# ssttuu/go-pbrt

Measured on AMD Instinct MI355X. Metric: Mpaths/s (samples×pixels/s) at 1920×1080, 64 spp; 1/2/4/8-GPU scaling + HBM GB/s vs roofline, higher is better.
Workload: dtype f64

## Files before the change

go-pbrt_amd/csrc/k_chain.h:

```cpp
#pragma once
#pragma clang fp contract(off)

#include "render_common.h"

namespace pbrtk {

template <bool kX>
__device__ __forceinline__ uint32_t ring_d(const Cursor& c, const SpecSampler& ss, uint32_t d) {
    if (!kX || c.rri < 0 || d == kBadExactD || c.rrn == 0) return d;
    return kRrFlag | (d == kBadSpecD ? kRrTailBad : d);
}

__device__ __forceinline__ int uni(int v) { return __builtin_amdgcn_readfirstlane(v); }
__device__ __forceinline__ uint32_t uni(uint32_t v) { return (uint32_t)__builtin_amdgcn_readfirstlane((int)v); }
__device__ __forceinline__ float uni(float v) { return __int_as_float(__builtin_amdgcn_readfirstlane(__float_as_int(v))); }
__device__ __forceinline__ uint64_t uni(uint64_t v) {
    return (uint64_t)uni((uint32_t)(v >> 32)) << 32 | uni((uint32_t)v);
}
__device__ __forceinline__ int64_t uni(int64_t v) { return (int64_t)uni((uint64_t)v); }
__device__ __forceinline__ CiGroup uni(const CiGroup& s) {
    CiGroup u;
    u.S = uni(s.S);
    u.pi = uni(s.pi);
    u.npx = uni(s.npx);
    u.A = uni(s.A);
    u.head = uni(s.head);
    u.nxt = uni(s.nxt);
    u.kh = uni(s.kh);
    u.phase = uni(s.phase);
    u.reissue = uni(s.reissue);
    u.rb0 = uni(s.rb0);
    u.rb1 = uni(s.rb1);
    u.nb = uni(s.nb);
    u.nnx = uni(s.nnx);
    u.nps = uni(s.nps);
    u.dcnt = uni(s.dcnt);
    u.dsum = uni(s.dsum);
    u.dsq = uni(s.dsq);
    return u;
}

template <int kW, int kDepth, bool kX, int kEu, bool kSpWin, bool kMulti>
__global__ __launch_bounds__(kWave * kW) __attribute__((amdgpu_waves_per_eu(kEu > 0 ? kEu : kDepth < 0 ? PBRT_CI_MESH_EU_WAVES : kX ? PBRT_CI_X_EU_WAVES : PBRT_CI_EU_WAVES, 8))) void k_chain_ci(
    DevScene sc, RenderParams rp, ChainLayout lay, const PcgJump* __restrict__ jump, WaveBufs wb, int64_t slot_base,
    int64_t nslots_batch, int lanes_per_tile, int ring_size, Counters* __restrict__ ctr,
    const uint32_t* __restrict__ order, uint32_t* __restrict__ ticks, int cstride, uint32_t* __restrict__ prog) {
    extern __shared__ __attribute__((aligned(16))) unsigned char lds[];
    const uint64_t t_begin = wall_clock64();
    if (prog && threadIdx.x == 0) __hip_atomic_fetch_add(&prog[0], 1u, __ATOMIC_RELAXED, __HIP_MEMORY_SCOPE_AGENT);
    const uint32_t cs = cstride == 1 ? 1u : 2u;
    constexpr int kT = kWave * kW;
    __shared__ uint16_t stack_lds[kDepth > 0 ? kDepth * kT : 1];
#ifdef PBRT_CI_DENSE_WALK
    __shared__ __attribute__((aligned(16))) unsigned char dense_lds[kDepth > 0 ? 16 : kW * kDenseScratch];
#endif
    __shared__ CiGroup gs[kCiMaxGroups];
    __shared__ uint64_t sh_state;
    __shared__ uint32_t sh_draws;
    __shared__ int sh_act;
    __shared__ int wcnt[kW];
#ifdef PBRT_CI_DIAG
    __shared__ uint32_t dh[64];
#endif
    static_assert(!kMulti || kW == 1, "several tiles per wave: one-wave workgroups only");
    const int tid = threadIdx.x, lane = tid & (kWave - 1), wv = kW > 1 ? uni(tid / kWave) : 0;
    stage_nodes(sc);
    const int L = kMulti ? lanes_per_tile : kT, G = kMulti ? kWave / L : 1;
    const int g = kMulti ? lane / L : 0, gl = kMulti ? lane - g * L : tid;
    const int64_t blk = order ? (int64_t)order[blockIdx.x] : (int64_t)blockIdx.x;
    const uint32_t R = (uint32_t)ring_size;
    const PcgJump& J = *jump;
    double* s1d = lay.s1d >= 0 ? (double*)(lds + lay.s1d) : nullptr;
    uint16_t* other = (uint16_t*)(lds + lay.other);
    uint32_t* vbuf = (uint32_t*)(lds + lay.vbuf);
    constexpr bool kNps = kW > 1 && !kX;
    const bool nps_on = kNps && rp.ci_nps != 0 && cstride == 1;
    constexpr uint32_t kNpsMinStats = 16;
    constexpr bool kStats = !kX && (kW > 1 || kDepth < 0);
    const float zcap = nps_on ? 3.0f : rp.ci_scap >= 0 ? 0.1f * (float)rp.ci_scap : kDepth < 0 ? 1.5f : 0.0f;
    auto ring_of = [&](int64_t pix) -> RingEnt* {
        return (RingEnt*)(lds + lay.ring) + (size_t)(nps_on ? (int)(pix & 1) : g) * R;
    };
    auto rpar = [&](int64_t pix) -> int { return nps_on ? (int)(pix & 1) : 0; };
    ChainCache* pcs = (ChainCache*)(lds + lay.pcs);
    uint16_t* stack = stack_lds + tid;
    const int n = rp.spp, ndims = rp.ndims;
#ifndef PBRT_CI_TAILCAP
#define PBRT_CI_TAILCAP 1
#endif
    const uint32_t dmax = (uint32_t)(camera_draws(ndims) + 8 * (rp.max_depth + 1) + 8);
    const pbrt_camera_desc& cam = *sc.camera;
    const unsigned long long gmask = !kMulti || L >= 64 ? ~0ULL : (((1ULL << (L & 63)) - 1ULL) << (g * L));
    const int64_t bs = blk * G + g;
    const uint64_t inc = pcg_inc_of((uint64_t)tile_of_slot(rp, slot_base + (bs < nslots_batch ? bs : 0)));
#ifdef PBRT_CI_DIAG
    unsigned long long steps = 0, busy = 0;
    unsigned long long ph_cyc[8] = {0, 0, 0, 0, 0, 0, 0, 0};
    long long tprev = clock64();
    auto mark = [&](int k) {
        long long now = clock64();
        ph_cyc[k] += (unsigned long long)(now - tprev);
        tprev = now;
    };
    if (tid < 64) dh[tid] = 0;
#define CI_DIAG(x) x
#else
    auto mark = [](int) {};
#define CI_DIAG(x)
#endif
    if (tid < G) {
        const int64_t b = blk * G + tid;
        CiGroup& s = gs[tid];
        s.pi = 0;
        s.kh = 1;
        s.A = s.head = s.nxt = 0;
        s.rb0 = s.rb1 = 0;
        s.nb = s.nnx = 0;
        s.nps = 0;
        s.dcnt = 0;
        s.dsum = s.dsq = 0.0f;
        s.reissue = 0;
        if (b < nslots_batch) {
            int64_t x0, y0, x1, y1;
            tile_bounds(rp, tile_of_slot(rp, slot_base + b), x0, y0, x1, y1);
            Pcg seed;
            pcg_seed(seed, (uint64_t)tile_of_slot(rp, slot_base + b));
            s.S = seed.state;
            s.npx = (x1 - x0) * (y1 - y0);
            s.phase = s.npx > 0 ? 0 : 2;
            wb.tile_npx[b] = 0;
        } else {
            s.S = 0;
            s.npx = 0;
            s.phase = 2;
        }
    }
    __syncthreads();

    uint32_t cancel_poll = 0;
    uint64_t last_host_poll = t_begin;
    uint32_t off = kNoOff;
    int opi_r = -1;
#ifdef PBRT_CI_LDS_STATE
    constexpr bool kLdsState = true;
#else
    constexpr bool kLdsState = kX;
#endif
    __shared__ Spec xs_beta[kLdsState ? kT : 1];
    __shared__ double xs_eta[kLdsState ? kT : 1];
    constexpr bool kStIssue = !kMulti;
    __shared__ uint64_t xs_st0[kLdsState && !kStIssue ? kT : 1];
    uint64_t st0_r = 0;
    Spec beta_r = spec(1);
    double eta_r = 1.0;
    uint64_t& st0 = [&]() -> uint64_t& { if constexpr (kLdsState && !kStIssue) return xs_st0[tid]; else return st0_r; }();
    Spec& beta = [&]() -> Spec& { if constexpr (kLdsState) return xs_beta[tid]; else return beta_r; }();
    double& eta_scale = [&]() -> double& { if constexpr (kLdsState) return xs_eta[tid]; else return eta_r; }();
    st0 = 0;
    beta = spec(1);
    eta_scale = 1.0;
    bool tracing = false;
    Cursor c;
    c.rri = -1;
    c.rrn = 0;
    c.rng.state = 0;
    c.rng.inc = inc;
    c.draws = 0;
    c.cur1d = c.cur2d = 0;
    c.k = -1;
    c.kdep = 0;
    int bounces = 1;
    Ray ray;
    ray.o = ray.d = V3{0, 0, 0};
    ray.tmax = kInf;
    ray.time = 0;

    CiGroup sg;
    if constexpr (kMulti) sg = gs[g];
    else sg = uni(gs[0]);
    int64_t rec = bs * wb.ppt + sg.pi;
    SpecSampler ss{wb.s1d + rec * wb.s1d_stride, n, ndims, kX && wb.rrb ? wb.rrb + bs * kCiMaxRing : nullptr};

    constexpr bool kOneScatter = kDepth >= 0 && !kSpWin;
    using Both = std::integral_constant<int, 0>;
    using Fresh = std::integral_constant<int, 1>;
    using Hits = std::integral_constant<int, 2>;
    int best = -1;
    V3 ph{0, 0, 0};
    auto traverse = [&]() __attribute__((always_inline)) {
        const int64_t opi = kNps ? (int64_t)opi_r : sg.pi;
        best = -1;
        int panic = 0;
#ifdef PBRT_CI_DENSE_WALK
        const bool dense = kDepth == 0 && sc.dense_ok && sc.use_lds_nodes;
        if (dense) bvh_walk_dense(sc, ray, tracing, panic, best, ph, dense_lds + (size_t)wv * kDenseScratch);
        if (tracing) {
            if (!dense) bvh_walk<false, kT, PBRT_CHAIN_LB, (kDepth < 0)>(sc, ray, stack, panic, best, ph);
#else
        if (tracing) {
            bvh_walk<false, kT, PBRT_CHAIN_LB, (kDepth < 0)>(sc, ray, stack, panic, best, ph);
#endif
            if (panic || best < 0) {
                RingEnt& e = ring_of(opi)[(off - (rpar(opi) ? sg.rb1 : sg.rb0)) & (R - 1u)];
                if constexpr (!kStIssue) e.st = st0;
                e.d = ring_d<kX>(c, ss, panic ? (c.k >= 0 ? kBadExactD : kBadSpecD) : c.draws);
                e.tag = off;
                off = kNoOff;
                tracing = false;
            }
        }
    };
    auto scatter = [&](auto which, bool fresh) __attribute__((always_inline)) {
        constexpr int kWhich = decltype(which)::value;
        const bool first = kWhich == Fresh::value ? true : kWhich == Hits::value ? false : fresh;
        if (kWhich == Fresh::value ? fresh : kWhich == Hits::value ? tracing : (fresh || tracing)) {
            const int64_t spi = kNps ? (int64_t)opi_r : sg.pi;
            SI si;
            BSDF b;
            BSDFX x;
            V3 wo = ray.d;
            bool ok = true;
            if (first) {
                const ChainCache& pc = pcs[2 * g + rpar(spi)];
                si = pc.si;
                b = pc.b;
                if constexpr (kX) x = pc.x;
                wo = pc.wo;
            } else {
                prim_si(sc, best, ray, ph, si);
                ok = (kX ? compute_bsdf_x(sc, si, b, x) : compute_bsdf(sc, si, b)) >= 0;
            }
            const int r = !ok ? 2
                              : traj_scatter<kX>(sc, si, b, x, wo, c, ss, beta, eta_scale, bounces, ray, rp.max_depth,
                                                 rp.rr_threshold);
            tracing = r == 0;
            if (r != 0) {
                RingEnt& e = ring_of(spi)[(off - (rpar(spi) ? sg.rb1 : sg.rb0)) & (R - 1u)];
                if constexpr (!kStIssue) e.st = st0;
                e.d = ring_d<kX>(c, ss, r == 1 ? c.draws : (c.k >= 0 ? kBadExactD : kBadSpecD));
                e.tag = off;
                off = kNoOff;
            }
        }
    };
    auto walk_drop = [&]() __attribute__((always_inline)) {
        const int64_t opi = kNps ? (int64_t)opi_r : sg.pi;
        __syncthreads();
        if (gl == 0 && sg.phase == 1) {
            CiGroup s = gs[g];
            if ((++cancel_poll & 127u) == 0) {
                const uint64_t now = wall_clock64();
                const bool host = now - last_host_poll >= 100000;
                if (host) last_host_poll = now;
                if (cancel_requested(sc, host)) s.phase = 2;
            }
            RingEnt* rcur = ring_of(s.pi);
            const uint32_t rbase = rpar(s.pi) ? s.rb1 : s.rb0;
            for (; s.phase == 1;) {
                RingEnt& e = rcur[(s.head - rbase) & (R - 1u)];
                if (e.tag != s.head) break;
                uint32_t d = e.d;
                if (kX && d < kBadExactD && (d & kRrFlag)) {
                    const RrBranches& b = ss.rrb[(s.head - rbase) & (R - 1u)];
                    d = (d & kRrTailBad) == kRrTailBad ? kBadSpecD : (d & kRrTailBad);
                    for (uint32_t i = 0; i < b.n; i++) {
                        const uint32_t cd = b.cd[i];
                        if (ss.s1d[(int)(cd & 0xFFu) * n + s.kh] < b.q[i]) {
                            d = cd >> 8;
                            break;
                        }
                    }
                }
                if (d == kBadSpecD) {
                    e.tag = kNoOff;
                    s.reissue = 1;
                    break;
                }
                wb.memb[rec * n + s.kh] = e.st;
                if (d == kBadExactD) {
                    wb.prec[rec].nvalid = s.kh + 1;
                    s.phase = 2;
                    break;
                }
                CI_DIAG(atomicAdd(&dh[min(d / 2u, 63u)], 1u);)
                CI_DIAG(if (d > dmax) ph_cyc[6]++;)
                CI_DIAG(if (d & 1u) atomicAdd(&ctr->odd_d, 1ull);)
                if (kStats) {
                    s.dcnt++;
                    s.dsum += (float)d;
                    s.dsq += (float)d * (float)d;
                }
                s.kh++;
                s.head += d;
                if (s.kh >= n) {
                    s.S = pcg_advance(J, s.S, inc, (uint64_t)(s.head - s.A));
                    s.A = s.head;
                    s.pi++;
                    s.phase = s.pi < s.npx ? 0 : 2;
                    break;
                }
            }
            if (s.nxt < s.head || (cs == 2u && ((s.nxt ^ s.head) & 1u))) s.nxt = s.head;
            int act = 0;
            const int left = n - s.kh;
            const bool stats = s.dcnt >= kNpsMinStats;
            if (nps_on && s.phase == 1 && !s.nps && (left == 1 || (stats && left <= rp.ci_nps)) &&
                s.pi + 1 < s.npx) {
                const PixelRec& pn = wb.prec[rec + 1];
                if (pn.hit && !pn.panic0) {
                    float lo = 0.0f;
                    if (left > 1) {
                        const float mu = s.dsum / (float)s.dcnt;
                        const float sd = sqrtf(fmaxf(0.0f, s.dsq / (float)s.dcnt - mu * mu));
                        lo = fmaxf(0.0f, (float)left * mu - 3.0f * sd * sqrtf((float)left));
                    }
                    s.nps = 1;
                    s.nb = s.head + (uint32_t)lo + (uint32_t)rp.sp_events;
                    s.nnx = s.nb;
                    if (rpar(s.pi + 1)) s.rb1 = s.nb;
                    else s.rb0 = s.nb;
                    act = 1;
                }
            }
            if (kNps) sh_act = act;
            CiGroup& gw = gs[g];
            gw.S = s.S;
            gw.A = s.A;
            gw.pi = s.pi;
            gw.head = s.head;
            gw.nxt = s.nxt;
            gw.kh = s.kh;
            gw.phase = s.phase;
            gw.reissue = s.reissue;
            if (kStats) {
                gw.dcnt = s.dcnt;
                gw.dsum = s.dsum;
                gw.dsq = s.dsq;
            }
            if (kNps) {
                gw.nps = s.nps;
                gw.nb = s.nb;
                gw.nnx = s.nnx;
                gw.rb0 = s.rb0;
                gw.rb1 = s.rb1;
            }
        }
        if (kNps && tid == 0 && !(gl == 0 && sg.phase == 1)) sh_act = 0;
        __syncthreads();
        if (kNps && sh_act) {
            const CiGroup s3 = uni(gs[0]);
            RingEnt* rn = ring_of(s3.pi + 1);
            for (uint32_t i = (uint32_t)tid; i < R; i += kT) rn[i].tag = kNoOff;
            if (tid == 0) {
                const PixelRec& pn = wb.prec[rec + 1];
                ChainCache& pc = pcs[2 * g + rpar(s3.pi + 1)];
                pc.si = pn.si;
                pc.b = pn.b;
                pc.wo = pn.wo;
                pc.hit = pn.hit;
            }
        }
        if (off != kNoOff) {
            const CiGroup s2 = gs[g];
            bool keep = false;
            if ((!kNps || opi == s2.pi) && s2.phase == 1)
                keep = !(off < s2.head || (cs == 2u && ((off ^ s2.head) & 1u)) ||
                         (PBRT_CI_TAILCAP && off > s2.head + (uint32_t)(n - 1 - s2.kh) * dmax));
            else if (kNps && opi == s2.pi && s2.phase == 0)
                keep = s2.nps != 0;
            else if (kNps && opi == s2.pi + 1 && s2.phase == 1)
                keep = s2.nps != 0;
            if (!keep) {
                off = kNoOff;
                tracing = false;
            }
        }
    };

    for (;;) {
        if constexpr (kOneScatter) {
            CI_DIAG(const unsigned long long tbusy = __ballot(tracing); if (lane == 0) busy += (unsigned long long)__popcll(tbusy);)
            traverse();
            mark(2);
            walk_drop();
            mark(4);
        }
        for (int q = 0; q < G; q++) {
            while (gs[q].phase == 0) {
                const int64_t bq = blk * G + q;
                const int64_t tile = tile_of_slot(rp, slot_base + bq);
                const uint64_t incq = pcg_inc_of((uint64_t)tile);
                const int64_t pi = gs[q].pi;
                const int64_t rec = bq * wb.ppt + pi;
                int64_t x0, y0, x1, y1;
                tile_bounds(rp, tile, x0, y0, x1, y1);
                const int64_t px = x0 + pi % (x1 - x0), py = y0 + pi / (x1 - x0);
                double* gs1d = wb.s1d + rec * wb.s1d_stride;
                double* sp = s1d ? s1d : gs1d;
                uint64_t S1;
                [[clang::always_inline]] S1 = start_pixel_wave<kSpWin>(rp, J, gs[q].S, incq, sp, other, vbuf, &sh_state, &sh_draws);
                if (s1d)
                    for (int idx = tid; idx < ndims * n; idx += kT) gs1d[idx] = s1d[idx];
                const double time_u = sp[1 < n ? 1 : 0];
                __syncthreads();
                const bool spec_ran = nps_on && gs[q].nps != 0;
                if (!spec_ran) {
                    RingEnt* rq = nps_on ? ring_of(pi) : (RingEnt*)(lds + lay.ring) + (size_t)q * R;
                    for (uint32_t i = (uint32_t)tid; i < R; i += kT) rq[i].tag = kNoOff;
                }
                PixelRec& pr = wb.prec[rec];
                const int hit0 = pr.hit, panic0 = pr.panic0;
                if (tid == 0) {
                    if (prog)
                        __hip_atomic_fetch_add(&prog[2], 1u, __ATOMIC_RELAXED, __HIP_MEMORY_SCOPE_AGENT);
                    const uint64_t now = wall_clock64();
                    const bool host = now - last_host_poll >= 100000;
                    if (host) last_host_poll = now;
                    if (cancel_requested(sc, host))
                        for (int q2 = 0; q2 < G; q2++) gs[q2].phase = 2;
                }
                if (tid == 0 && gs[q].phase == 0) {
                    if (hit0)
                        pr.si.time = camera_ray(cam, (double)px, (double)py, time_u, V2{0.0, 0.0}).time;
                    ChainCache& pq = pcs[2 * q + rpar(pi)];
                    pq.si = pr.si;
                    pq.b = pr.b;
                    if constexpr (kX) pq.x = pr.x;
                    pq.wo = pr.wo;
                    pq.hit = hit0;
                    CiGroup& s = gs[q];
                    s.S = S1;
                    s.A += sh_draws;
                    s.head = s.A;
                    s.nxt = (spec_ran && s.A >= s.nb) ? max(s.nnx, s.A) : s.A;
                    if (!spec_ran) {
                        if (rpar(pi)) s.rb1 = s.A;
                        else s.rb0 = s.A;
                    }
                    s.nps = 0;
                    s.kh = 1;
                    s.reissue = 0;
                    wb.tile_npx[bq] = (int32_t)(pi + 1);
                    if (panic0) {
                        s.phase = 2;
                    } else if (hit0) {
                        s.phase = 1;
                    } else {
                        if (ndims < 2) {
                            s.S = pcg_advance(J, S1, incq, (uint64_t)(n - 1) * camera_draws(ndims));
                            s.A += (uint32_t)(n - 1) * camera_draws(ndims);
                        }
                        s.pi = pi + 1;
                        s.phase = s.pi < s.npx ? 0 : 2;
                    }
                }
                __syncthreads();
            }
        }
        mark(0);
        bool any_chain = false;
        for (int q = 0; q < G; q++) any_chain |= gs[q].phase == 1;
        if (!any_chain) break;
        CI_DIAG(steps++;)

        if constexpr (kMulti) sg = gs[g];
        else sg = uni(gs[0]);
        rec = bs * wb.ppt + sg.pi;
        ss.s1d = wb.s1d + rec * wb.s1d_stride;
        bool fresh = false;
        {
            const bool idle = sg.phase == 1 && off == kNoOff;
            const unsigned long long m = __ballot(idle) & gmask;
            int nidle = __popcll(m);
            int rank;
            if constexpr (kMulti) rank = __popcll(m & ((1ULL << lane) - 1ULL));
            else rank = (int)__builtin_amdgcn_mbcnt_hi((uint32_t)(m >> 32), __builtin_amdgcn_mbcnt_lo((uint32_t)m, 0u));
            if (kW > 1) {
                if (lane == 0) wcnt[wv] = nidle;
                __syncthreads();
                int before = 0, tot = 0;
                for (int w = 0; w < kW; w++) {
                    const int cw = wcnt[w];
                    before += w < wv ? cw : 0;
                    tot += cw;
                }
                rank += before;
                nidle = tot;
            }
            const int re = (sg.reissue && nidle > 0) ? 1 : 0;
            const uint32_t nx0 = sg.nxt;
            const int avail = nx0 < sg.head + R ? (int)((sg.head + R - nx0 + cs - 1) / cs) : 0;
#if PBRT_CI_TAILCAP
            const uint32_t tail = sg.head + (uint32_t)(n - 1 - sg.kh) * dmax;
            const int capn = nx0 <= tail ? (int)((tail - nx0) / cs) + 1 : 0;
            int nspec = min(min(nidle - re, avail), capn);
            if (kStats && zcap > 0.0f && sg.dcnt >= kNpsMinStats) {
                const float rem = (float)(n - 1 - sg.kh);
                const float mu = sg.dsum / (float)sg.dcnt;
                const float sd = sqrtf(fmaxf(0.0f, sg.dsq / (float)sg.dcnt - mu * mu));
                const uint32_t scap = sg.head + (uint32_t)(rem * mu + zcap * sd * sqrtf(rem));
                nspec = min(nspec, nx0 <= scap ? (int)((scap - nx0) / cs) + 1 : 0);
            }
#else
            const int nspec = min(nidle - re, avail);
#endif
            int nspec1 = 0;
            if (kNps && sg.phase == 1 && sg.nps) {
                const int avail1 = sg.nnx < sg.nb + R ? (int)(sg.nb + R - sg.nnx) : 0;
                nspec1 = max(0, min(nidle - re - max(nspec, 0), avail1));
            }
            uint32_t o = kNoOff;
            bool exact = false;
            int opix = (int)sg.pi;
            if (idle) {
                if (re && rank == 0) {
                    o = sg.head;
                    exact = true;
                } else {
                    rank -= re;
                    if (rank < nspec) {
                        o = nx0 + cs * (uint32_t)rank;
                    } else if (kNps && rank - nspec < nspec1) {
                        o = sg.nnx + (uint32_t)(rank - nspec);
                        opix = (int)sg.pi + 1;
                    }
                }
            }
            if (gl == 0 && sg.phase == 1) {
                gs[g].nxt = nx0 + cs * (uint32_t)max(nspec, 0);
                if (kNps) gs[g].nnx = sg.nnx + (uint32_t)nspec1;
                CI_DIAG(ph_cyc[5] += (unsigned long long)(max(nspec, 0) + nspec1 + re);)
                CI_DIAG(ph_cyc[7] += (unsigned long long)nspec1;)
                if (re) gs[g].reissue = 0;
            }
            if (o != kNoOff) {
                off = o;
                if (kNps) opi_r = opix;
                RingEnt& e = ring_of(opix)[(off - (rpar(opix) ? sg.rb1 : sg.rb0)) & (R - 1u)];
                if constexpr (kStIssue) {
                    const uint64_t st = pcg_advance(J, sg.S, inc, (uint64_t)(o - sg.A));
                    e.st = st;
                    c.rng.state = st;
                } else {
                    st0 = pcg_advance(J, sg.S, inc, (uint64_t)(o - sg.A));
                    c.rng.state = st0;
                }
                c.draws = 0;
                c_camera(c, ndims);
                c.k = exact ? sg.kh : -1;
                c.kdep = 0;
                if constexpr (kX) {
                    c.rri = (!exact && ss.rrb) ? (int)((off - sg.rb0) & (R - 1u)) : -1;
                    c.rrn = 0;
                }
                beta = spec(1);
                eta_scale = 1.0;
                bounces = 1;
                fresh = true;
            }
        }
        if constexpr (kOneScatter) {
            mark(1);
            scatter(Both{}, fresh);
            mark(3);
        } else {
            scatter(Fresh{}, fresh);
            mark(1);
            CI_DIAG(const unsigned long long tbusy = __ballot(tracing); if (lane == 0) busy += (unsigned long long)__popcll(tbusy);)
            traverse();
            mark(2);
            scatter(Hits{}, false);
            mark(3);
            walk_drop();
            mark(4);
        }
    }
#ifdef PBRT_CI_DIAG
    __syncthreads();
    if (tid < 64 && dh[tid]) atomicAdd(&ctr->dhist[tid], (unsigned long long)dh[tid]);
    if (tid == 0) {
        atomicAdd(&ctr->windows, steps);
        for (int k = 0; k < 8; k++) atomicAdd(&ctr->phase[k], ph_cyc[k]);
        atomicAdd(&ctr->nps_issued, ph_cyc[7]);
    }
    if (lane == 0) atomicAdd(&ctr->busy, busy);
#endif
#undef CI_DIAG
    if (prog) {
        __threadfence();
        __syncthreads();
    }
    if (tid == 0) {
        if (prog && G == 1 && bs < nslots_batch) {
// ... 16 lines not shown
```

go-pbrt_amd/csrc/k_chain_c.hip:

```cpp
#pragma clang fp contract(off)

#include "render_common.h"
#include "cam_sample.h"
#include "k_chain.h"

namespace pbrtk {

#ifndef PBRT_CAM_EU_WAVES
#define PBRT_CAM_EU_WAVES 3
#endif

struct CamGroup {
    uint64_t S;
    int64_t pi;
    int64_t npx;
    uint32_t A;
    uint32_t head;
    uint32_t nxt;
    int kh;
    int phase;
    int px, py;
};

__global__ __launch_bounds__(kWave) __attribute__((amdgpu_waves_per_eu(PBRT_CAM_EU_WAVES, 8))) void k_chain_cam(
    DevScene sc, RenderParams rp, ChainLayout lay, const PcgJump* __restrict__ jump, WaveBufs wb, int64_t slot_base,
    int64_t nslots_batch, const uint32_t* __restrict__ order, uint32_t* __restrict__ ticks) {
    extern __shared__ __attribute__((aligned(16))) unsigned char lds[];
    const uint64_t t_begin = wall_clock64();
    __shared__ uint16_t stack_lds[1];
    __shared__ CamGroup gs;
    __shared__ uint64_t sh_state;
    __shared__ uint32_t sh_draws;
    const int tid = threadIdx.x;
    stage_nodes(sc);
    const int64_t bs = order ? (int64_t)order[blockIdx.x] : (int64_t)blockIdx.x;
    if (bs >= nslots_batch) return;
    constexpr uint32_t R = kCiRingBytes / sizeof(RingEnt);
    const PcgJump& J = *jump;
    double* s1d = lay.s1d >= 0 ? (double*)(lds + lay.s1d) : nullptr;
    uint16_t* other = (uint16_t*)(lds + lay.other);
    uint32_t* vbuf = (uint32_t*)(lds + lay.vbuf);
    RingEnt* ring = (RingEnt*)(lds + lay.ring);
    uint16_t* stack = stack_lds + tid;
    const int n = rp.spp, ndims = rp.ndims;
    const uint32_t dmax = pbrtcam::cam_draws(ndims) + (uint32_t)(8 * (rp.max_depth + 1) + 8);
    const pbrt_camera_desc& cam = *sc.camera;
    const int64_t tile = tile_of_slot(rp, slot_base + bs);
    const uint64_t inc = pcg_inc_of((uint64_t)tile);
    int64_t x0, y0, x1, y1;
    tile_bounds(rp, tile, x0, y0, x1, y1);
    if (tid == 0) {
        Pcg seed;
        pcg_seed(seed, (uint64_t)tile);
        gs.S = seed.state;
        gs.pi = 0;
        gs.npx = (x1 - x0) * (y1 - y0);
        gs.A = gs.head = gs.nxt = 0;
        gs.kh = 1;
        gs.phase = (gs.npx > 0 && n > 1) ? 0 : 2;
        gs.px = gs.py = 0;
        wb.tile_npx[bs] = 0;
    }
    __syncthreads();

    uint32_t cancel_poll = 0;
    uint64_t last_host_poll = t_begin;
    uint32_t off = kNoOff;
    bool tracing = false;
    Cursor c;
    c.rri = -1;
    c.rrn = 0;
    c.rng.state = 0;
    c.rng.inc = inc;
    c.draws = 0;
    c.cur1d = c.cur2d = 0;
    c.k = -1;
    c.kdep = 0;
    Spec beta = spec(1);
    double eta_scale = 1.0;
    int bounces = 1;
    Ray ray;
    ray.o = ray.d = V3{0, 0, 0};
    ray.tmax = kInf;
    ray.time = 0;
    const SpecSampler ss{nullptr, n, ndims, nullptr};

    auto finish = [&](uint32_t d) {
        RingEnt& e = ring[off & (R - 1u)];
        e.d = d;
        e.tag = off;
        off = kNoOff;
        tracing = false;
    };

    for (;;) {
        if (tracing) {
            int panic = 0, best = -1;
            V3 ph{0, 0, 0};
            bvh_walk<false, kWave, PBRT_CHAIN_LB, false>(sc, ray, stack, panic, best, ph);
            if (panic || best < 0) {
                finish(panic ? kBadExactD : c.draws);
            } else {
                SI si;
                BSDF b;
                BSDFX x;
                const V3 wo = ray.d;
                prim_si(sc, best, ray, ph, si);
                const int r = compute_bsdf(sc, si, b) < 0
                                  ? 2
                                  : traj_scatter<false>(sc, si, b, x, wo, c, ss, beta, eta_scale, bounces, ray,
                                                        rp.max_depth, rp.rr_threshold);
                if (r != 0) finish(r == 1 ? c.draws : kBadExactD);
            }
        }
        __syncthreads();
        if (tid == 0 && gs.phase == 1) {
            CamGroup s = gs;
            if ((++cancel_poll & 127u) == 0) {
                const uint64_t now = wall_clock64();
                const bool host = now - last_host_poll >= 100000;
                if (host) last_host_poll = now;
                if (cancel_requested(sc, host)) s.phase = 2;
            }
            const int64_t rec = bs * wb.ppt + s.pi;
            for (; s.phase == 1;) {
                const RingEnt& e = ring[s.head & (R - 1u)];
                if (e.tag != s.head) break;
                const uint32_t d = e.d;
                wb.memb[rec * n + s.kh] = e.st;
                if (d == kBadExactD) {
                    wb.prec[rec].nvalid = s.kh + 1;
                    s.phase = 2;
                    break;
                }
                s.kh++;
                s.head += d;
                if (s.kh >= n) {
                    s.S = pcg_advance(J, s.S, inc, (uint64_t)(s.head - s.A));
                    s.A = s.head;
                    s.pi++;
                    s.phase = s.pi < s.npx ? 0 : 2;
                    break;
                }
            }
            if (s.nxt < s.head) s.nxt = s.head;
            gs.S = s.S;
            gs.A = s.A;
            gs.pi = s.pi;
            gs.head = s.head;
            gs.nxt = s.nxt;
            gs.kh = s.kh;
            gs.phase = s.phase;
        }
        __syncthreads();
        if (off != kNoOff) {
            const uint32_t head = uni(gs.head);
            const bool keep = uni(gs.phase) == 1 && off >= head && off <= head + (uint32_t)(n - 1 - uni(gs.kh)) * dmax;
            if (!keep) {
                off = kNoOff;
                tracing = false;
            }
        }
        while (gs.phase == 0) {
            const int64_t pi = gs.pi;
            const int64_t rec = bs * wb.ppt + pi;
            uint64_t S1 = gs.S;
            uint32_t sp_draws = 0;
            if (ndims > 0) {
                double* gs1d = wb.s1d + rec * wb.s1d_stride;
                [[clang::always_inline]] S1 = start_pixel_wave<false>(rp, J, gs.S, inc, s1d ? s1d : gs1d, other, vbuf, &sh_state, &sh_draws);
                sp_draws = sh_draws;
                if (s1d)
                    for (int idx = tid; idx < ndims * n; idx += kWave) gs1d[idx] = s1d[idx];
            }
            __syncthreads();
            for (uint32_t i = (uint32_t)tid; i < R; i += kWave) ring[i].tag = kNoOff;
            if (tid == 0) {
                const uint64_t now = wall_clock64();
                const bool host = now - last_host_poll >= 100000;
                if (host) last_host_poll = now;
                PixelRec& pr = wb.prec[rec];
                pr.hit = 1;
                pr.panic0 = 0;
                pr.nvalid = n;
                wb.tile_npx[bs] = (int32_t)(pi + 1);
                gs.S = S1;
                gs.A += sp_draws;
                gs.head = gs.nxt = gs.A;
                gs.kh = 1;
                gs.px = (int)(x0 + pi % (x1 - x0));
                gs.py = (int)(y0 + pi / (x1 - x0));
                gs.phase = cancel_requested(sc, host) ? 2 : 1;
            }
            __syncthreads();
        }
        if (gs.phase != 1) break;

        {
            const uint32_t head = uni(gs.head), nx0 = uni(gs.nxt), A = uni(gs.A);
            const int kh = uni(gs.kh);
            const uint64_t S = uni(gs.S);
            const int px = uni(gs.px), py = uni(gs.py);
            const bool idle = off == kNoOff;
            const unsigned long long m = __ballot(idle);
            const int nidle = __popcll(m);
            const int rank = (int)__builtin_amdgcn_mbcnt_hi((uint32_t)(m >> 32), __builtin_amdgcn_mbcnt_lo((uint32_t)m, 0u));
            const int avail = nx0 < head + R ? (int)(head + R - nx0) : 0;
            const uint32_t tail = head + (uint32_t)(n - 1 - kh) * dmax;
            const int capn = nx0 <= tail ? (int)(tail - nx0) + 1 : 0;
            const int nspec = min(min(nidle, avail), capn);
            if (tid == 0) gs.nxt = nx0 + (uint32_t)nspec;
            if (idle && rank < nspec) {
                off = nx0 + (uint32_t)rank;
                uint64_t st = pcg_advance(J, S, inc, (uint64_t)(off - A));
                ring[off & (R - 1u)].st = st;
                const pbrtcam::CamSample cs = pbrtcam::cam_sample(st, inc, ndims);
                c.rng.state = st;
                c.draws = cs.draws;
                c.cur1d = ndims < 1 ? ndims : 1;
                c.cur2d = ndims < 2 ? ndims : 2;
                c.kdep = 0;
                beta = spec(1);
                eta_scale = 1.0;
                bounces = 1;
                if (bounces >= rp.max_depth) {
                    finish(c.draws);
                } else {
                    ray = camera_ray(cam, (double)px + cs.film_x, (double)py + cs.film_y, cs.time_u,
                                     V2{cs.lens_x, cs.lens_y});
                    tracing = true;
                }
            }
        }
    }
    if (tid == 0 && ticks) {
        const uint64_t t_end = wall_clock64();
        ticks[bs] = (uint32_t)min(t_end - t_begin, (uint64_t)0xFFFFFFFFu);
    }
}

}
```

go-pbrt_amd/csrc/pbrt_spec.h:

```cpp
#pragma once
#pragma clang fp contract(off)

#include "pbrt_path.h"
#include <type_traits>

namespace pbrt {

struct PcgJump {
    uint64_t a[64];
    uint64_t b[64];
};
__device__ __forceinline__ uint64_t pcg_advance(const PcgJump& J, uint64_t s, uint64_t inc, uint64_t n) {
    for (int i = 0; n; ++i, n >>= 1)
        if (n & 1) s = J.a[i] * s + inc * J.b[i];
    return s;
}
__device__ __forceinline__ uint32_t pcg_output(uint64_t old) {
    uint32_t xs = (uint32_t)(((old >> 18) ^ old) >> 27);
    uint32_t rot = (uint32_t)(old >> 59);
    return (xs >> rot) | (xs << ((rot + 1u) & 31u));
}

constexpr int kRrBranches = 3;
struct RrBranches {
    double q[kRrBranches];
    uint32_t cd[kRrBranches];
    uint32_t n;
};
struct SpecSampler {
    const double* s1d;
    int spp, ndims;
    RrBranches* rrb;
};
struct Cursor {
    Pcg rng;
    uint32_t draws;
    int cur1d, cur2d;
    int k;
    int kdep;
    int rri;
    int rrn;
};
__device__ __forceinline__ double c_get1d(Cursor& c, const SpecSampler& s) {
    if (c.cur1d < s.ndims) {
        const int d = c.cur1d++;
        if (c.k < 0) {
            c.kdep = 1;
            return 0.5;
        }
        return s.s1d[d * s.spp + c.k];
    }
    c.draws++;
    return pcg_float(c.rng);
}
__device__ __forceinline__ void c_skip1d(Cursor& c, const SpecSampler& s) {
    if (c.cur1d < s.ndims) {
        c.cur1d++;
        return;
    }
    c.draws++;
    pcg_next(c.rng);
}
__device__ __forceinline__ V2 c_get2d(Cursor& c, const SpecSampler& s) {
    if (c.cur2d < s.ndims) {
        c.cur2d++;
        return V2{0.0, 0.0};
    }
    c.draws += 2;
    double x = pcg_float(c.rng);
// ... 153 lines not shown
        if (kX && type == -1) {
            panic = PBRT_PANIC_NIL_DEREF;
            return true;
        }
        if (is_black(f) || pdf == 0.0) {
            done = true;
        } else {
            double wp = absdot(wi, isect.sn) / pdf;
            s.beta = smul(s.beta, smuls(f, wp));
            if (kX && (type & BXDF_SPECULAR) && (type & BXDF_TRANSMISSION)) {
                const double eta = x.eta;
                if (dot(wo, isect.n) > 0) s.eta_scale *= eta * eta;
                else s.eta_scale *= 1 / (eta * eta);
            }
            s.ray.o = offset_ray_origin(isect.p, isect.perr, isect.n, wi);
            s.ray.d = wi;
            s.ray.tmax = kInf;
            s.ray.time = isect.time;
            Spec rr = smuls(s.beta, kX ? s.eta_scale : 1.0);
            if (max_component(rr) < rr_threshold && s.bounces > 3) {
                double q = gomath::max(0.05, 1 - max_component(rr));
                double u1 = c_get1d(c, ss);
                if (c.kdep || u1 < q) done = true;
                else s.beta = sdivs(s.beta, 1 - q);
            }
        }
    }
    if (pending) {
        Spec ld = spec(0);
        if (shadow) {
            add_rays(s, kRayShadow);
            const bool occluded = bvh_traverse<true, PBRT_PATHS_LB>(sc, sr, nullptr, stack, panic);
            if (panic) return true;
            if (!occluded) {
                if constexpr (kLdsAux) ld = s.aux[1];
                else ld = ld_vis;
            }
        }
        if (max_component(ld) > 10) {
            panic = PBRT_PANIC_LD_GT_10;
            return true;
        }
        if constexpr (kLdsAux) beta0 = s.aux[0];
        add_L(s, smul(beta0, ld));
    }
    return done;
}

template <bool kX = false>
__device__ inline int traj_scatter(const DevScene& sc, const SI& isect, const BSDF& b, const BSDFX& x, V3 wo,
                                   Cursor& c, const SpecSampler& ss, Spec& beta, double& eta_scale, int& bounces,
                                   Ray& ray, int max_depth, double rr_threshold) {
    if ((kX ? bsdfx_nonspecular(b, x) : b.n_bxdfs > 0) && sc.n_lights > 0) {
        c_skip1d(c, ss);
        c_get2d(c, ss);
        c_get2d(c, ss);
    }
    V2 u = c_get2d(c, ss);
    V3 wi;
    double pdf;
    int type = 0;
    Spec f = kX ? bsdfx_sample_f(b, x, wo, u, wi, pdf, type) : bsdf_sample_f(b, wo, u, wi, pdf);
    if (kX && type == -1) return 2;
    if (is_black(f) || pdf == 0.0) return 1;
    double wp = absdot(wi, isect.sn) / pdf;
    beta = smul(beta, smuls(f, wp));
    if (kX && (type & BXDF_SPECULAR) && (type & BXDF_TRANSMISSION)) {
        const double eta = x.eta;
        if (dot(wo, isect.n) > 0) eta_scale *= eta * eta;
        else eta_scale *= 1 / (eta * eta);
    }
    ray.o = offset_ray_origin(isect.p, isect.perr, isect.n, wi);
    ray.d = wi;
    ray.tmax = kInf;
    ray.time = isect.time;
    Spec rr = smuls(beta, kX ? eta_scale : 1.0);
    if (max_component(rr) < rr_threshold && bounces > 3) {
        double q = gomath::max(0.05, 1 - max_component(rr));
        if (kX && c.k < 0 && c.rri >= 0 && c.cur1d < ss.ndims) {
            RrBranches& rb = ss.rrb[c.rri];
            if (c.rrn == kRrBranches || c.draws >= (1u << 24)) return 2;
            rb.q[c.rrn] = q;
            rb.cd[c.rrn] = (c.draws << 8) | (uint32_t)c.cur1d;
            rb.n = (uint32_t)++c.rrn;
            c.cur1d++;
            beta = sdivs(beta, 1 - q);
        } else {
            double u1 = c_get1d(c, ss);
            if (c.kdep) return 2;
            if (u1 < q) return 1;
            beta = sdivs(beta, 1 - q);
        }
    }
    bounces++;
    return bounces >= max_depth ? 1 : 0;
}

}
```

go-pbrt_amd/csrc/render.hip:

```cpp
#pragma clang fp contract(off)

#include <hip/hip_runtime.h>

#include <algorithm>
#include <atomic>
#include <chrono>
#include <cstdio>
#include <cstring>
#include <string>
#include <functional>
#include <mutex>
#include <unordered_map>
#include <vector>

#include "../../include/pbrt_gpu.h"
#include "../../include/pbrt_diag.h"
#include "../../include/pbrt_scene.h"
#include "mesh_bvh.h"
#include "query_buffers.h"
#include "render_kernels.h"

using namespace pbrt;
using namespace pbrtk;

// ... 436 lines not shown
        v[i].prim_to_world = p.prim_to_world;
        v[i].kind = p.kind;
        v[i].material = p.material;
        v[i].prim_identity = is_identity(p.prim_to_world.m) ? 1 : 0;
        v[i].fast = xf_fast_kind(p.prim_to_world.m_inv) | xf_fast_kind(v[i].shape.object_to_world.m_inv) << 8;
    }
    return v;
}

int validate_scene(const pbrt_scene_desc* s) {
    if (!s) return PBRT_E_INVALID;
    if (s->n_prims < 0 || s->n_nodes < 0 || s->n_lights < 0 || s->n_shapes < 0 || s->n_materials < 0)
        return PBRT_E_INVALID;
    if (s->n_nodes > 32767) return PBRT_E_UNSUPPORTED;
    for (int i = 0; i < s->n_prims; i++) {
        const pbrt_primitive_desc& p = s->prims[i];
        if (p.shape < 0 || p.shape >= s->n_shapes || p.material < 0 || p.material >= s->n_materials)
            return PBRT_E_INVALID;
        if (p.kind != PBRT_PRIM_GEOMETRIC && p.kind != PBRT_PRIM_TRANSFORMED) return PBRT_E_INVALID;
    }
    for (int i = 0; i < s->n_shapes; i++)
        if (s->shapes[i].type != PBRT_SHAPE_SPHERE && s->shapes[i].type != PBRT_SHAPE_DISK) return PBRT_E_UNSUPPORTED;
    for (int i = 0; i < s->n_nodes; i++) {
        const pbrt_bvh_node& n = s->nodes[i];
        if (n.n_prims > 0 && (int64_t)n.offset + n.n_prims > s->n_prims) return PBRT_E_INVALID;
        if (n.n_prims == 0 && (n.offset >= (uint32_t)s->n_nodes || n.axis > 2)) return PBRT_E_INVALID;
    }
    for (int i = 0; i < s->n_materials; i++)
        if (s->materials[i].type < PBRT_MAT_MATTE || s->materials[i].type > PBRT_MAT_GLASS) return PBRT_E_UNSUPPORTED;
    if (s->n_meshes < 0 || (s->n_meshes > 0 && !s->meshes)) return PBRT_E_INVALID;
    for (int i = 0; i < s->n_meshes; i++) {
        const pbrt_mesh_desc& m = s->meshes[i];
        if (m.n_vertices < 0 || m.n_triangles < 0 || m.material < 0 || m.material >= s->n_materials ||
            (m.n_triangles > 0 && (!m.p || !m.indices)))
            return PBRT_E_INVALID;
        for (int64_t k = 0; k < 3 * (int64_t)m.n_triangles; k++)
            if (m.indices[k] < 0 || m.indices[k] >= m.n_vertices) return PBRT_E_INVALID;
    }
    for (int i = 0; i < s->n_lights; i++) {
        const pbrt_light_desc& l = s->lights[i];
        if (l.type < PBRT_LIGHT_POINT || l.type > PBRT_LIGHT_DIFFUSE_AREA) return PBRT_E_UNSUPPORTED;
        if (l.type == PBRT_LIGHT_DIFFUSE_AREA &&
            (l.shape < 0 || l.shape >= s->n_shapes || s->shapes[l.shape].type != PBRT_SHAPE_SPHERE))
            return PBRT_E_UNSUPPORTED;
    }
    const pbrt_film_desc& f = s->film;
    if (f.crop_max_x <= f.crop_min_x || f.crop_max_y <= f.crop_min_y) return PBRT_E_INVALID;
    return PBRT_OK;
}

const PcgJump& pcg_jump_table() {
    static PcgJump J = [] {
        PcgJump t;
        uint64_t a = 0x5851f42d4c957f2dULL, b = 1;
        for (int i = 0; i < 64; i++) {
            t.a[i] = a;
            t.b[i] = b;
            b = b * (a + 1);
            a = a * a;
        }
        return t;
    }();
    return J;
}

int paths_ci_pixels(const pbrt_gpu_ctx* c, const RenderParams& rp);
bool paths_wf_enabled(const pbrt_gpu_ctx* c);
#ifndef PBRT_SP_SERIAL_KB
#define PBRT_SP_SERIAL_KB 4
#endif
#ifndef PBRT_SP_WINDOW_KB
#define PBRT_SP_WINDOW_KB 6
#endif
#ifndef PBRT_CI_STAGE_KB
#define PBRT_CI_STAGE_KB 8
#endif
bool wave_eligible(const pbrt_gpu_ctx* c, const pbrt_render_desc* rd, const RenderParams& rp, ChainLayout& L,
                   ChainLayout& Lci) {
    if (rd->flags & PBRT_FLAG_PANIC_FIDELITY) return false;
    const bool dl = rd->integrator == PBRT_INTEGRATOR_DIRECT_LIGHTING;
    if (c->non_matte && (c->rough_glass || (dl && rd->max_depth > 64) ||
                         (!dl && (c->host_scene.n_nodes > kLdsNodes ||
                                  (!paths_wf_enabled(c) && paths_ci_pixels(c, rp) > 0 && paths_ci_pixels(c, rp) < 4)))))
        return false;
    if (dl) {
        if (rd->n_dims < 1 || (rd->n_dims < 2 && c->host_scene.camera.lens_radius > 0)) return false;
    } else if (rd->integrator != PBRT_INTEGRATOR_PATH || rd->max_depth > 2048) {
        return false;
    } else if (rd->n_dims < 2 && !(rd->n_dims == 1 && c->host_scene.camera.lens_radius == 0)) {
        return false;
    }
    const int nl = c->host_scene.n_lights;
    if (!dl && nl > kMaxCachedLights) return false;
    if (!dl && nl > 0) {
        const pbrt_distribution_desc& d = c->host_dist;
        if (!(d.func_int > 0)) return false;
        for (int i = 0; i < d.count; i++)
            if (!(d.func[i] > 0)) return false;
    }
    if ((size_t)film_lds_bytes(rp) + kFilmThreads * sizeof(int) > c->lds_per_block) return false;
    const int64_t n = rp.spp, nd = rp.ndims;
    if (n > 4096 || nd * n > 8192) return false;
    int64_t off = 0;
    auto put = [&](int64_t bytes) {
        int64_t o = off;
        off += (bytes + 15) & ~int64_t(15);
        return (int)o;
    };
    L.s1d = put(nd * n * 8);
    L.other = put(nd * n * 2);
    L.sbuf = put(kWave * 8);
    L.dbuf = put(kWave * 4);
    L.vbuf = put(sp_vbuf_bytes(rp));
// ... 1576 lines not shown
```

go-pbrt_amd/csrc/render_common.h:

```cpp

#pragma once
#pragma clang fp contract(off)

#include <hip/hip_runtime.h>

#include <cstdint>

#include "../../include/pbrt_gpu.h"
#include "../../include/pbrt_scene.h"
#include "mesh_bvh.h"
#include "pbrt_spec.h"

namespace pbrtk {

using namespace pbrt;


constexpr int kWave = 64;

struct RenderParams {
    int64_t film_min_x, film_min_y, film_w, film_h;
    int64_t tile_size, ntx, nty;
    int64_t tile_begin, tile_stride, n_slots;
    int64_t slot_w, slot_h;
// ... 634 lines not shown
            }
        }
        if (2 * i + 1 < rp.max_depth) {
            g2();
            g2();
        }
    }
    return d;
}
__device__ __forceinline__ uint32_t dl_draws(const RenderParams& rp, int hit, int n_lights) {
    return dl_chain_draws(rp, hit ? 1 : 0, n_lights);
}
constexpr int kProbes = 2;
constexpr double kCostPixel = 150.0;

#ifndef PBRT_CI_MESH_EU_WAVES
#define PBRT_CI_MESH_EU_WAVES 3
#endif
#ifndef PBRT_CI_EU_WAVES
#define PBRT_CI_EU_WAVES 3
#endif
#ifndef PBRT_CI_X_EU_WAVES
#define PBRT_CI_X_EU_WAVES 2
#endif
#ifndef PBRT_CHAIN_LB
#define PBRT_CHAIN_LB 1
#endif
constexpr uint32_t kNoOff = 0xFFFFFFFFu;
constexpr uint32_t kNoSlot = 0xFFFFFFFFu;
constexpr int kProgHead = 3;
constexpr uint32_t kBadSpecD = 0xFFFFFFFEu;
constexpr uint32_t kBadExactD = 0xFFFFFFFDu;
struct RingEnt {
    uint32_t tag;
    uint32_t d;
    uint64_t st;
};
struct CiGroup {
    uint64_t S;
    int64_t pi;
    int64_t npx;
    uint32_t A;
    uint32_t head;
    uint32_t nxt;
    int kh;
    int phase;
    int reissue;
    uint32_t rb0, rb1;
    uint32_t nb, nnx;
    int nps;
    uint32_t dcnt;
    float dsum, dsq;
};

}
```

Before: 380.6.

## Carry PCG states incrementally and use precomputed near-step jump tables

Replaces the per-issue log-depth pcg_advance from the group anchor with carried states (Sn, Sq) kept in the group struct. These are advanced by small offsets through new precomputed step and mid tables (pcg_step, pcg_advance_near). The PcgJump table grows with 128+8 affine maps, and a compile-time pcg_skip path is added behind a macro for skipped light draws. It cuts the serial 64-bit multiply chains on the issue and walk paths, at the cost of more shared state, a larger jump table read from memory, and subtle correctness risk in the rank offset bookkeeping across waves.

```diff
diff --git a/go-pbrt_amd/csrc/k_chain.h b/go-pbrt_amd/csrc/k_chain.h
--- a/go-pbrt_amd/csrc/k_chain.h
+++ b/go-pbrt_amd/csrc/k_chain.h
@@ -39,6 +39,13 @@
     u.dsq = uni(s.dsq);
     return u;
 }
+__device__ __forceinline__ CiGroupC uni(const CiGroupC& s) {
+    CiGroupC u;
+    static_cast<CiGroup&>(u) = uni(static_cast<const CiGroup&>(s));
+    u.Sn = uni(s.Sn);
+    u.Sq = uni(s.Sq);
+    return u;
+}
 
 template <int kW, int kDepth, bool kX, int kEu, bool kSpWin, bool kMulti>
 __global__ __launch_bounds__(kWave * kW) __attribute__((amdgpu_waves_per_eu(kEu > 0 ? kEu : kDepth < 0 ? PBRT_CI_MESH_EU_WAVES : kX ? PBRT_CI_X_EU_WAVES : PBRT_CI_EU_WAVES, 8))) void k_chain_ci(
@@ -54,7 +61,8 @@
 #ifdef PBRT_CI_DENSE_WALK
     __shared__ __attribute__((aligned(16))) unsigned char dense_lds[kDepth > 0 ? 16 : kW * kDenseScratch];
 #endif
-    __shared__ CiGroup gs[kCiMaxGroups];
+    using Group = std::conditional_t<kMulti, CiGroup, CiGroupC>;
+    __shared__ Group gs[kMulti ? kCiMaxGroups : 1];
     __shared__ uint64_t sh_state;
     __shared__ uint32_t sh_draws;
     __shared__ int sh_act;
@@ -110,7 +118,7 @@
 #endif
     if (tid < G) {
         const int64_t b = blk * G + tid;
-        CiGroup& s = gs[tid];
+        Group& s = gs[tid];
         s.pi = 0;
         s.kh = 1;
         s.A = s.head = s.nxt = 0;
@@ -120,6 +128,7 @@
         s.dcnt = 0;
         s.dsum = s.dsq = 0.0f;
         s.reissue = 0;
+        if constexpr (!kMulti) s.Sn = s.Sq = 0;
         if (b < nslots_batch) {
             int64_t x0, y0, x1, y1;
             tile_bounds(rp, tile_of_slot(rp, slot_base + b), x0, y0, x1, y1);
@@ -149,6 +158,8 @@
     __shared__ Spec xs_beta[kLdsState ? kT : 1];
     __shared__ double xs_eta[kLdsState ? kT : 1];
     constexpr bool kStIssue = !kMulti;
+    constexpr bool kCarry = !kMulti;
+    static_assert(!kCarry || kStIssue, "the carried states rely on ring entries that hold their state from the issue on");
     __shared__ uint64_t xs_st0[kLdsState && !kStIssue ? kT : 1];
     uint64_t st0_r = 0;
     Spec beta_r = spec(1);
@@ -175,7 +186,7 @@
     ray.tmax = kInf;
     ray.time = 0;
 
-    CiGroup sg;
+    Group sg;
     if constexpr (kMulti) sg = gs[g];
     else sg = uni(gs[0]);
     int64_t rec = bs * wb.ppt + sg.pi;
@@ -256,6 +267,8 @@
             }
             RingEnt* rcur = ring_of(s.pi);
             const uint32_t rbase = rpar(s.pi) ? s.rb1 : s.rb0;
+            uint32_t dl = 0;
+            bool walked = false;
             for (; s.phase == 1;) {
                 RingEnt& e = rcur[(s.head - rbase) & (R - 1u)];
                 if (e.tag != s.head) break;
@@ -292,15 +305,24 @@
                 }
                 s.kh++;
                 s.head += d;
+                dl = d;
+                walked = true;
                 if (s.kh >= n) {
-                    s.S = pcg_advance(J, s.S, inc, (uint64_t)(s.head - s.A));
+                    if constexpr (kCarry) s.S = pcg_advance_near(J, e.st, inc, (uint64_t)d);
+                    else s.S = pcg_advance(J, s.S, inc, (uint64_t)(s.head - s.A));
                     s.A = s.head;
                     s.pi++;
                     s.phase = s.pi < s.npx ? 0 : 2;
                     break;
                 }
             }
-            if (s.nxt < s.head || (cs == 2u && ((s.nxt ^ s.head) & 1u))) s.nxt = s.head;
+            if (s.nxt < s.head || (cs == 2u && ((s.nxt ^ s.head) & 1u))) {
+                s.nxt = s.head;
+                if constexpr (kCarry)
+                    if (s.phase == 1)
+                        gs[g].Sn = walked ? pcg_advance_near(J, rcur[(s.head - dl - rbase) & (R - 1u)].st, inc, (uint64_t)dl)
+                                      : pcg_advance(J, s.S, inc, (uint64_t)(s.head - s.A));
+            }
             int act = 0;
             const int left = n - s.kh;
             const bool stats = s.dcnt >= kNpsMinStats;
@@ -317,6 +339,7 @@
                     s.nps = 1;
                     s.nb = s.head + (uint32_t)lo + (uint32_t)rp.sp_events;
                     s.nnx = s.nb;
+                    if constexpr (kNps) gs[g].Sq = pcg_advance_near(J, s.S, inc, (uint64_t)(s.nb - s.A));
                     if (rpar(s.pi + 1)) s.rb1 = s.nb;
                     else s.rb0 = s.nb;
                     act = 1;
@@ -348,7 +371,7 @@
         if (kNps && tid == 0 && !(gl == 0 && sg.phase == 1)) sh_act = 0;
         __syncthreads();
         if (kNps && sh_act) {
-            const CiGroup s3 = uni(gs[0]);
+            const CiGroup s3 = uni(static_cast<const CiGroup&>(gs[0]));
             RingEnt* rn = ring_of(s3.pi + 1);
             for (uint32_t i = (uint32_t)tid; i < R; i += kT) rn[i].tag = kNoOff;
             if (tid == 0) {
@@ -428,11 +451,12 @@
                     if constexpr (kX) pq.x = pr.x;
                     pq.wo = pr.wo;
                     pq.hit = hit0;
-                    CiGroup& s = gs[q];
+                    Group& s = gs[q];
                     s.S = S1;
                     s.A += sh_draws;
                     s.head = s.A;
                     s.nxt = (spec_ran && s.A >= s.nb) ? max(s.nnx, s.A) : s.A;
+                    if constexpr (kCarry) s.Sn = s.nxt == s.A ? S1 : s.Sq;
                     if (!spec_ran) {
                         if (rpar(pi)) s.rb1 = s.A;
                         else s.rb0 = s.A;
@@ -473,6 +497,7 @@
             const unsigned long long m = __ballot(idle) & gmask;
             int nidle = __popcll(m);
             int rank;
+            int wbefore = 0;
             if constexpr (kMulti) rank = __popcll(m & ((1ULL << lane) - 1ULL));
             else rank = (int)__builtin_amdgcn_mbcnt_hi((uint32_t)(m >> 32), __builtin_amdgcn_mbcnt_lo((uint32_t)m, 0u));
             if (kW > 1) {
@@ -484,8 +509,13 @@
                     before += w < wv ? cw : 0;
                     tot += cw;
                 }
+                if constexpr (kCarry) {
+                    before = uni(before);
+                    tot = uni(tot);
+                }
                 rank += before;
                 nidle = tot;
+                wbefore = before;
             }
             const int re = (sg.reissue && nidle > 0) ? 1 : 0;
             const uint32_t nx0 = sg.nxt;
@@ -509,9 +539,22 @@
                 const int avail1 = sg.nnx < sg.nb + R ? (int)(sg.nb + R - sg.nnx) : 0;
                 nspec1 = max(0, min(nidle - re - max(nspec, 0), avail1));
             }
+            const int ns = max(nspec, 0);
+            const int r0 = max(wbefore - re, 0), r0c = min(r0, ns), r0q = r0 - r0c;
+            uint64_t wSn = 0, wSq = 0, nSn = 0, nSq = 0;
+            if constexpr (kCarry) {
+                wSn = nSn = sg.Sn;
+                wSq = nSq = sg.Sq;
+                if (ns > 0) nSn = pcg_advance_near(J, sg.Sn, inc, (uint64_t)(cs * (uint32_t)ns));
+                if (kNps && nspec1 > 0) nSq = pcg_advance_near(J, sg.Sq, inc, (uint64_t)nspec1);
+                if (kW > 1 && r0c > 0) wSn = pcg_advance_near(J, sg.Sn, inc, (uint64_t)(cs * (uint32_t)r0c));
+                if (kNps && r0q > 0 && nspec1 > 0) wSq = pcg_advance_near(J, sg.Sq, inc, (uint64_t)r0q);
+            }
             uint32_t o = kNoOff;
             bool exact = false;
             int opix = (int)sg.pi;
+            uint32_t kst = 0;
+            uint64_t wbase = wSn;
             if (idle) {
                 if (re && rank == 0) {
                     o = sg.head;
@@ -520,15 +563,20 @@
                     rank -= re;
                     if (rank < nspec) {
                         o = nx0 + cs * (uint32_t)rank;
+                        kst = cs * (uint32_t)(rank - r0c);
                     } else if (kNps && rank - nspec < nspec1) {
                         o = sg.nnx + (uint32_t)(rank - nspec);
                         opix = (int)sg.pi + 1;
+                        kst = (uint32_t)(rank - nspec - r0q);
+                        wbase = wSq;
                     }
                 }
             }
             if (gl == 0 && sg.phase == 1) {
                 gs[g].nxt = nx0 + cs * (uint32_t)max(nspec, 0);
+                if constexpr (kCarry) gs[g].Sn = nSn;
                 if (kNps) gs[g].nnx = sg.nnx + (uint32_t)nspec1;
+                if constexpr (kNps) gs[g].Sq = nSq;
                 CI_DIAG(ph_cyc[5] += (unsigned long long)(max(nspec, 0) + nspec1 + re);)
                 CI_DIAG(ph_cyc[7] += (unsigned long long)nspec1;)
                 if (re) gs[g].reissue = 0;
@@ -537,8 +585,10 @@
                 off = o;
                 if (kNps) opi_r = opix;
                 RingEnt& e = ring_of(opix)[(off - (rpar(opix) ? sg.rb1 : sg.rb0)) & (R - 1u)];
-                if constexpr (kStIssue) {
-                    const uint64_t st = pcg_advance(J, sg.S, inc, (uint64_t)(o - sg.A));
+                if constexpr (kCarry) {
+                    const uint64_t st = exact    ? e.st
+                                        : kW == 1 ? pcg_step(J, wbase, inc, kst)
+                                                  : pcg_advance_near(J, wbase, inc, (uint64_t)kst);
                     e.st = st;
                     c.rng.state = st;
                 } else {
diff --git a/go-pbrt_amd/csrc/k_chain_c.hip b/go-pbrt_amd/csrc/k_chain_c.hip
--- a/go-pbrt_amd/csrc/k_chain_c.hip
+++ b/go-pbrt_amd/csrc/k_chain_c.hip
@@ -17,6 +17,7 @@
     uint32_t A;
     uint32_t head;
     uint32_t nxt;
+    uint64_t Sn;
     int kh;
     int phase;
     int px, py;
@@ -56,6 +57,7 @@
         gs.pi = 0;
         gs.npx = (x1 - x0) * (y1 - y0);
         gs.A = gs.head = gs.nxt = 0;
+        gs.Sn = 0;
         gs.kh = 1;
         gs.phase = (gs.npx > 0 && n > 1) ? 0 : 2;
         gs.px = gs.py = 0;
@@ -123,6 +125,8 @@
                 if (cancel_requested(sc, host)) s.phase = 2;
             }
             const int64_t rec = bs * wb.ppt + s.pi;
+            uint32_t dl = 0;
+            bool walked = false;
             for (; s.phase == 1;) {
                 const RingEnt& e = ring[s.head & (R - 1u)];
                 if (e.tag != s.head) break;
@@ -135,15 +139,22 @@
                 }
                 s.kh++;
                 s.head += d;
+                dl = d;
+                walked = true;
                 if (s.kh >= n) {
-                    s.S = pcg_advance(J, s.S, inc, (uint64_t)(s.head - s.A));
+                    s.S = pcg_advance_near(J, e.st, inc, (uint64_t)d);
                     s.A = s.head;
                     s.pi++;
                     s.phase = s.pi < s.npx ? 0 : 2;
                     break;
                 }
             }
-            if (s.nxt < s.head) s.nxt = s.head;
+            if (s.nxt < s.head) {
+                s.nxt = s.head;
+                if (s.phase == 1)
+                    gs.Sn = walked ? pcg_advance_near(J, ring[(s.head - dl) & (R - 1u)].st, inc, (uint64_t)dl)
+                                   : pcg_advance(J, s.S, inc, (uint64_t)(s.head - s.A));
+            }
             gs.S = s.S;
             gs.A = s.A;
             gs.pi = s.pi;
@@ -187,6 +198,7 @@
                 gs.S = S1;
                 gs.A += sp_draws;
                 gs.head = gs.nxt = gs.A;
+                gs.Sn = S1;
                 gs.kh = 1;
                 gs.px = (int)(x0 + pi % (x1 - x0));
                 gs.py = (int)(y0 + pi / (x1 - x0));
@@ -197,9 +209,9 @@
         if (gs.phase != 1) break;
 
         {
-            const uint32_t head = uni(gs.head), nx0 = uni(gs.nxt), A = uni(gs.A);
+            const uint32_t head = uni(gs.head), nx0 = uni(gs.nxt);
             const int kh = uni(gs.kh);
-            const uint64_t S = uni(gs.S);
+            const uint64_t Sn = uni(gs.Sn);
             const int px = uni(gs.px), py = uni(gs.py);
             const bool idle = off == kNoOff;
             const unsigned long long m = __ballot(idle);
@@ -209,10 +221,14 @@
             const uint32_t tail = head + (uint32_t)(n - 1 - kh) * dmax;
             const int capn = nx0 <= tail ? (int)(tail - nx0) + 1 : 0;
             const int nspec = min(min(nidle, avail), capn);
-            if (tid == 0) gs.nxt = nx0 + (uint32_t)nspec;
+            const uint64_t nSn = nspec > 0 ? pcg_advance_near(J, Sn, inc, (uint64_t)nspec) : Sn;
+            if (tid == 0) {
+                gs.nxt = nx0 + (uint32_t)nspec;
+                gs.Sn = nSn;
+            }
             if (idle && rank < nspec) {
                 off = nx0 + (uint32_t)rank;
-                uint64_t st = pcg_advance(J, S, inc, (uint64_t)(off - A));
+                uint64_t st = pcg_step(J, Sn, inc, (uint32_t)rank);
                 ring[off & (R - 1u)].st = st;
                 const pbrtcam::CamSample cs = pbrtcam::cam_sample(st, inc, ndims);
                 c.rng.state = st;
diff --git a/go-pbrt_amd/csrc/pbrt_spec.h b/go-pbrt_amd/csrc/pbrt_spec.h
--- a/go-pbrt_amd/csrc/pbrt_spec.h
+++ b/go-pbrt_amd/csrc/pbrt_spec.h
@@ -2,19 +2,11 @@
 #pragma clang fp contract(off)
 
 #include "pbrt_path.h"
+#include "pcg_jump.h"
 #include <type_traits>
 
 namespace pbrt {
 
-struct PcgJump {
-    uint64_t a[64];
-    uint64_t b[64];
-};
-__device__ __forceinline__ uint64_t pcg_advance(const PcgJump& J, uint64_t s, uint64_t inc, uint64_t n) {
-    for (int i = 0; n; ++i, n >>= 1)
-        if (n & 1) s = J.a[i] * s + inc * J.b[i];
-    return s;
-}
 __device__ __forceinline__ uint32_t pcg_output(uint64_t old) {
     uint32_t xs = (uint32_t)(((old >> 18) ^ old) >> 27);
     uint32_t rot = (uint32_t)(old >> 59);
@@ -274,9 +266,21 @@
                                    Cursor& c, const SpecSampler& ss, Spec& beta, double& eta_scale, int& bounces,
                                    Ray& ray, int max_depth, double rr_threshold) {
     if ((kX ? bsdfx_nonspecular(b, x) : b.n_bxdfs > 0) && sc.n_lights > 0) {
+#ifdef PBRT_TRAJ_SKIP_MAP
+        int k = 0;
+        if (c.cur1d < ss.ndims) c.cur1d++;
+        else k += 1;
+        for (int i = 0; i < 2; i++) {
+            if (c.cur2d < ss.ndims) c.cur2d++;
+            else k += 2;
+        }
+        c.draws += (uint32_t)k;
+        c.rng.state = pcg_skip(c.rng.state, c.rng.inc, k);
+#else
         c_skip1d(c, ss);
         c_get2d(c, ss);
         c_get2d(c, ss);
+#endif
     }
     V2 u = c_get2d(c, ss);
     V3 wi;
diff --git a/go-pbrt_amd/csrc/pcg_jump.h b/go-pbrt_amd/csrc/pcg_jump.h
--- /dev/null
+++ b/go-pbrt_amd/csrc/pcg_jump.h
@@ -0,0 +1,84 @@
+#pragma once
+
+#include <stdint.h>
+
+#if defined(__HIPCC__)
+#define PBRT_PCG_HD __host__ __device__ __forceinline__
+#else
+#define PBRT_PCG_HD inline
+#endif
+
+namespace pbrt {
+
+constexpr uint64_t kPcgMult = 0x5851f42d4c957f2dULL;
+constexpr int kPcgNear = 128;
+constexpr int kPcgMid = 8;
+
+struct PcgStep {
+    uint64_t a, b;
+};
+struct PcgJump {
+    uint64_t a[64];
+    uint64_t b[64];
+    alignas(16) PcgStep step[kPcgNear];
+    PcgStep mid[kPcgMid];
+};
+
+PBRT_PCG_HD void pcg_jump_fill(PcgJump& t) {
+    uint64_t a = kPcgMult, b = 1;
+    for (int i = 0; i < 64; i++) {
+        t.a[i] = a;
+        t.b[i] = b;
+        b = b * (a + 1);
+        a = a * a;
+    }
+    PcgStep m{1, 0};
+    for (int k = 0; k < kPcgNear * kPcgMid; k++) {
+        if (k < kPcgNear) t.step[k] = m;
+        if (k % kPcgNear == 0) t.mid[k / kPcgNear] = m;
+        m.a = m.a * kPcgMult;
+        m.b = m.b * kPcgMult + 1;
+    }
+}
+
+PBRT_PCG_HD uint64_t pcg_advance(const PcgJump& J, uint64_t s, uint64_t inc, uint64_t n) {
+    for (int i = 0; n; ++i, n >>= 1)
+        if (n & 1) s = J.a[i] * s + inc * J.b[i];
+    return s;
+}
+PBRT_PCG_HD uint64_t pcg_step(const PcgJump& J, uint64_t s, uint64_t inc, uint32_t k) {
+    const PcgStep m = J.step[k];
+    return m.a * s + inc * m.b;
+}
+PBRT_PCG_HD uint64_t pcg_advance_near(const PcgJump& J, uint64_t s, uint64_t inc, uint64_t n) {
+    if (n < (uint64_t)kPcgNear) return pcg_step(J, s, inc, (uint32_t)n);
+    if (n < (uint64_t)(kPcgNear * kPcgMid)) {
+        const PcgStep m = J.mid[n / kPcgNear];
+        return pcg_step(J, m.a * s + inc * m.b, inc, (uint32_t)(n % kPcgNear));
+    }
+    return pcg_advance(J, s, inc, n);
+}
+
+constexpr int kPcgSkipMax = 5;
+constexpr PcgStep pcg_const_map(int k) {
+    PcgStep m{1, 0};
+    for (int i = 0; i < k; i++) {
+        m.a = m.a * kPcgMult;
+        m.b = m.b * kPcgMult + 1;
+    }
+    return m;
+}
+PBRT_PCG_HD uint64_t pcg_skip(uint64_t s, uint64_t inc, int k) {
+    constexpr PcgStep m1 = pcg_const_map(1), m2 = pcg_const_map(2), m3 = pcg_const_map(3), m4 = pcg_const_map(4),
+                      m5 = pcg_const_map(5);
+    switch (k) {
+    case 0: return s;
+    case 1: return m1.a * s + inc * m1.b;
+    case 2: return m2.a * s + inc * m2.b;
+    case 3: return m3.a * s + inc * m3.b;
+    case 4: return m4.a * s + inc * m4.b;
+    default: return m5.a * s + inc * m5.b;
+    }
+}
+
+}
diff --git a/go-pbrt_amd/csrc/render.hip b/go-pbrt_amd/csrc/render.hip
--- a/go-pbrt_amd/csrc/render.hip
+++ b/go-pbrt_amd/csrc/render.hip
@@ -512,13 +512,7 @@
 const PcgJump& pcg_jump_table() {
     static PcgJump J = [] {
         PcgJump t;
-        uint64_t a = 0x5851f42d4c957f2dULL, b = 1;
-        for (int i = 0; i < 64; i++) {
-            t.a[i] = a;
-            t.b[i] = b;
-            b = b * (a + 1);
-            a = a * a;
-        }
+        pcg_jump_fill(t);
         return t;
     }();
     return J;
diff --git a/go-pbrt_amd/csrc/render_common.h b/go-pbrt_amd/csrc/render_common.h
--- a/go-pbrt_amd/csrc/render_common.h
+++ b/go-pbrt_amd/csrc/render_common.h
@@ -710,5 +710,8 @@
     uint32_t dcnt;
     float dsum, dsq;
 };
-
-}
+struct CiGroupC : CiGroup {
+    uint64_t Sn, Sq;
+};
+
+}
```

New measurement: 387.6 (median of 6 runs). 1.02x the previous value.
